# zdebruine/RcppML

Hardware: AMD Instinct MI355X
Metric: ALS updates/sec (cols solved/s), k=64 sparse NMF (higher is better)
Workload: dtype f32; 1 GPU; configs[1]: simulateNMF 20000x100000 (x1 GPUs, column shards) 1%-dense CSC, k=64, MSE, coordinate-descent NNLS (cd_maxit=100, cd_tol=1e-8), L1 row normalisation, loss every iteration; rows=20000, cols_per_gpu=100000, nnz_per_gpu=20054852, k=64, solver=cd, cd_variant=auto, parallelism=column-shard x1

## Files before the change

### rcppml_amd/csrc/cd_placement.hip.h

```cpp
#pragma once
#include <cstdint>

namespace rk {

struct CdPlace {
    int simds;
    int rounds;
    int desc;
    int extra_top;
};

constexpr int CD_PLACE_DESC = 0x6;
constexpr int CD_PLACE_EXTRA_TOP = 0;

__host__ __device__ inline int64_t cd_place_pos(const CdPlace& pl, int g, int r) {
    return (int64_t)r * pl.simds + (((pl.desc >> r) & 1) ? pl.simds - 1 - g : g);
}
__host__ __device__ inline int64_t cd_place_extra(const CdPlace& pl, int g) { return pl.extra_top ? pl.simds - 1 - g : g; }

__host__ __device__ inline int64_t cd_place_unserp(int64_t p, int tpb, int64_t ncols) {
    const int64_t blk = p / tpb, grp = blk >> 4;
    if ((grp & 1) && (grp + 1) * 16 <= (ncols >> 7)) return (((grp << 4) + 15 - (blk & 15)) * tpb) + p % tpb;
    return p;
}

}
```

### rcppml_amd/csrc/kernels_cd_mfma.hip.h

```cpp
#pragma once
#include "kernels.hip.h"
#include "cd_placement.hip.h"

namespace rk {


struct CdStepOut { float a, nx; };

__device__ __forceinline__ float cd_max_nc(float a, float b, float inf) { return __builtin_amdgcn_fmed3f(a, b, inf); }

template <bool SIMPLE>
__device__ __forceinline__ CdStepOut cd_scalar_step(float b, float xo, float ginv, bool active, float l1_cd, float l2_cd,
                                                    float lo, float hi) {
    CdStepOut o;
    if constexpr (SIMPLE) {
        const float diff = b * ginv;
        o.a = __builtin_fmaxf(diff, -xo);
        o.nx = __builtin_fmaxf(xo + diff, 0.f);
    } else {
        float diff = b * ginv;
        diff -= l1_cd;
        diff = __builtin_fmaf(l2_cd, xo, diff);
        const float nv = xo + diff;
        const bool neg = nv < lo, up = nv > hi;
        float nx = neg ? lo : (up ? hi : nv);
        float a = neg ? lo - xo : (up ? hi - xo : diff);
        const bool on = active && (ginv > 0.f);
        a = on ? a : 0.f;
        nx = on ? nx : xo;
        o.a = a;
        o.nx = nx;
    }
    return o;
}

__host__ __device__ constexpr size_t cd_mfma_lds_bytes(int RT) {
    return RT <= 2 ? (size_t)(16 * RT) * 64 * sizeof(float4) : ((size_t)(32 * RT) * (32 * RT) + 2 * (32 * RT)) * sizeof(float);
}

template <int RT>
__device__ __forceinline__ void cd_mfma_fill_lds(const float* __restrict__ G , int k) {
    constexpr int KP = 32 * RT;
    constexpr bool PACK = RT <= 2;
    extern __shared__ __attribute__((aligned(16))) char smem_raw[];
    float* Gs = reinterpret_cast<float*>(smem_raw);
    float2* tab_s = reinterpret_cast<float2*>(Gs + KP * KP);
    float4* img = reinterpret_cast<float4*>(smem_raw);
    {
        auto gp = [&](int col, int row) { return (row < k && col < k) ? G[(int64_t)col * k + row] : (row == col ? 1.f : 0.f); };
        if constexpr (PACK) {
            for (int e = threadIdx.x; e < (KP / 2) * 64; e += blockDim.x) {
                const int pr = e >> 6, w6 = e & 63;
                const int i = 2 * pr + (w6 >> 5), r = w6 & 31;
                const int h = (r >> 2) & 1, v = (r & 3) + 4 * (r >> 3);
                const float gd = gp(i, i);
                float4 t;
                t.x = -gp(i, 2 * v + h);
                t.y = RT == 2 ? -gp(i, 32 + 2 * v + h) : 0.f;
                t.z = gd > 0.f ? 1.f / gd : 0.f;
                t.w = (i & 1) ? gp(i - 1, i) : 0.f;
                img[e] = t;
            }
        } else {
            for (int e = threadIdx.x; e < KP * KP; e += blockDim.x) {
                const int pr = e >> 6, w6 = e & 63;
                const int i = 2 * (pr / RT) + (w6 >> 5), rt = pr % RT, r = w6 & 31;
                const int h = (r >> 2) & 1, v = (r & 3) + 4 * (r >> 3);
                Gs[e] = -gp(i, 32 * rt + 2 * v + h);
            }
            for (int i = threadIdx.x; i < KP; i += blockDim.x) {
                float2 t;
                const float gd = gp(i, i);
                t.x = gd > 0.f ? 1.f / gd : 0.f;
                t.y = (i & 1) ? gp(i - 1, i) : 0.f;
                tab_s[i] = t;
            }
        }
    }
}

template <int RT, int CT, bool SIMPLE>
__device__ __forceinline__ void cd_mfma_tile(const int64_t base, const float* __restrict__ B, float* __restrict__ X, int k, int64_t ncols,
                                             float l1_pre, int warm, int zero_init, float l1_cd, float l2_cd, int nonneg, int maxit,
                                             float tol, float ub_cd, float ub_post, int* __restrict__ sweeps,
                                             const int* __restrict__ order, unsigned long long* __restrict__ stats) {
    constexpr int KP = 32 * RT;
    constexpr bool PACK = RT <= 2;
    constexpr float XSIGN = SIMPLE ? -1.f : 1.f;
    extern __shared__ __attribute__((aligned(16))) char smem_raw[];
    float* Gs = reinterpret_cast<float*>(smem_raw);
    float2* tab_s = reinterpret_cast<float2*>(Gs + KP * KP);
    float4* img = reinterpret_cast<float4*>(smem_raw);
    const int lane = threadIdx.x & 63;
    const int half = lane >> 5, cl = lane & 31;
    if (base >= ncols) return;
    int64_t j[CT];
    bool inb[CT];
#pragma unroll
    for (int ct = 0; ct < CT; ++ct) {
        const int64_t slot = base + ct * 32 + cl;
        inb[ct] = slot < ncols;
        j[ct] = (inb[ct] && order) ? order[slot] : slot;
    }
    f32x16 acc[RT][CT];
    float xr[RT][CT][16];
#pragma unroll
    for (int rt = 0; rt < RT; ++rt)
#pragma unroll
        for (int ct = 0; ct < CT; ++ct) {
            const float* bj = B + j[ct] * (int64_t)k;
            const float* xj = X + j[ct] * (int64_t)k;
#pragma unroll
            for (int v = 0; v < 16; ++v) {
                const int row = 32 * rt + 2 * v + half;
                const bool ok = inb[ct] && row < k;
                float bv = ok ? bj[row] : 0.f;
                if (ok && l1_pre != 0.f) bv -= l1_pre;
                acc[rt][ct][v] = bv;
                xr[rt][ct][v] = (ok && !zero_init) ? XSIGN * xj[row] : 0.f;
            }
        }
    struct PairOps { float av[RT]; float ginv, coup; };
    auto load_pair = [&](int p) {
        PairOps o;
        if constexpr (PACK) {
            const float4 t = img[p * 64 + lane];
            o.av[0] = t.x;
            if constexpr (RT == 2) o.av[1] = t.y;
            o.ginv = t.z; o.coup = t.w;
        } else {
#pragma unroll
            for (int rt2 = 0; rt2 < RT; ++rt2) o.av[rt2] = Gs[(p * RT + rt2) * 64 + lane];
            const float2 t = tab_s[2 * p + half];
            o.ginv = t.x; o.coup = t.y;
        }
        return o;
    };
    if (warm) {
#pragma unroll
        for (int rt = 0; rt < RT; ++rt)
#pragma unroll
            for (int q = 0; q < 16; ++q) {
                const int i = 32 * rt + 2 * q;
                const PairOps po = load_pair(i >> 1);
#pragma unroll
                for (int rt2 = 0; rt2 < RT; ++rt2) {
#pragma unroll
                    for (int ct = 0; ct < CT; ++ct)
                        acc[rt2][ct] = __builtin_amdgcn_mfma_f32_32x32x2f32(po.av[rt2], XSIGN * xr[rt][ct][q], acc[rt2][ct], 0, 0, 0);
                }
            }
    }
    const float lo = nonneg ? 0.f : -INFINITY;
    const float hi = ub_cd > 0.f ? ub_cd : INFINITY;
    const bool check = tol > 0.f;
    const float inv_k = 1.f / static_cast<float>(k);
    bool active[CT];
    int nsweep[CT];
#pragma unroll
    for (int ct = 0; ct < CT; ++ct) { active[ct] = inb[ct]; nsweep[ct] = 0; }
    PairOps cur = load_pair(0);
    for (int it = 0; it < maxit; ++it) {
        bool any_active = false;
#pragma unroll
        for (int ct = 0; ct < CT; ++ct) any_active |= active[ct];
        if (!__any(any_active)) break;
        float tsum[CT];
#pragma unroll
        for (int ct = 0; ct < CT; ++ct) { tsum[ct] = 0.f; nsweep[ct] += active[ct] ? 1 : 0; }
#pragma unroll
        for (int rt = 0; rt < RT; ++rt)
#pragma unroll
            for (int q = 0; q < 16; ++q) {
                constexpr int KPc = KP;
                const int inext = (32 * rt + 2 * q + 2) % KPc;
                const int rtn = (q == 15 ? rt + 1 : rt) % RT;
                const PairOps nxt = load_pair(inext >> 1);
                const float g_oe = cur.coup;
                float aval[CT];
#pragma unroll
                for (int ct = 0; ct < CT; ++ct) {
                    const float b = acc[rt][ct][q];
                    const float xo = xr[rt][ct][q];
                    if constexpr (SIMPLE) {
                        const float ginv = cur.ginv;
                        float ae_lo = cd_max_nc(b * ginv, xo, hi);
                        asm volatile("s_nop 1\n\tv_permlane32_swap_b32 %0, %0" : "+v"(ae_lo));
                        const float bo = __builtin_fmaf(-g_oe, ae_lo, b);
                        const float diff = bo * ginv;
                        const float a = cd_max_nc(diff, xo, hi);
                        const float nxn = __builtin_fminf(xo - diff, 0.f);
                        aval[ct] = a;
                        xr[rt][ct][q] = nxn;
                        tsum[ct] = __builtin_fmaf(tabs(a), __builtin_amdgcn_rcpf(tabs(nxn) + 1e-15f), tsum[ct]);
                    } else {
                        const float ginv = cur.ginv;
                        const CdStepOut e = cd_scalar_step<SIMPLE>(b, xo, ginv, active[ct], l1_cd, l2_cd, lo, hi);
                        float ae_lo = e.a;
                        asm volatile("s_nop 1\n\tv_permlane32_swap_b32 %0, %0" : "+v"(ae_lo));
                        const float bo = __builtin_fmaf(-g_oe, ae_lo, b);
                        const CdStepOut o = cd_scalar_step<SIMPLE>(bo, xo, ginv, active[ct], l1_cd, l2_cd, lo, hi);
                        aval[ct] = o.a;
                        xr[rt][ct][q] = o.nx;
                        tsum[ct] = __builtin_fmaf(tabs(o.a), __builtin_amdgcn_rcpf(tabs(o.nx) + 1e-15f), tsum[ct]);
                    }
                }
#pragma unroll
                for (int s2 = 0; s2 < RT; ++s2) {
                    const int rt2 = (rtn + s2) % RT;
#pragma unroll
                    for (int ct = 0; ct < CT; ++ct)
                        acc[rt2][ct] = __builtin_amdgcn_mfma_f32_32x32x2f32(cur.av[rt2], aval[ct], acc[rt2][ct], 0, 0, 0);
                }
                cur = nxt;
                __builtin_amdgcn_sched_barrier(0);
            }
        bool froze = false;
#pragma unroll
        for (int ct = 0; ct < CT; ++ct) {
            const float tot = tsum[ct] + __shfl_xor(tsum[ct], 32, 64);
            const bool now = active[ct] && !(check && tot * inv_k < tol);
            froze |= active[ct] && !now;
            active[ct] = now;
        }
        if constexpr (SIMPLE) {
            if (__any(froze)) {
#pragma unroll
                for (int rt = 0; rt < RT; ++rt)
#pragma unroll
                    for (int ct = 0; ct < CT; ++ct)
#pragma unroll
                        for (int v = 0; v < 16; ++v) acc[rt][ct][v] = active[ct] ? acc[rt][ct][v] : 0.f;
            }
        }
    }
#pragma unroll
    for (int ct = 0; ct < CT; ++ct) {
        if (!inb[ct]) continue;
        float* xj = X + j[ct] * (int64_t)k;
#pragma unroll
        for (int rt = 0; rt < RT; ++rt)
#pragma unroll
            for (int v = 0; v < 16; ++v) {
                const int row = 32 * rt + 2 * v + half;
                if (row < k) {
                    float val = SIMPLE ? 0.f - xr[rt][ct][v] : xr[rt][ct][v];
                    if (ub_post > 0.f) val = val < ub_post ? val : ub_post;
                    xj[row] = val;
                }
            }
        if (sweeps && half == 0) sweeps[j[ct]] = nsweep[ct];
    }
    int nsw = 0, ncol = 0;
#pragma unroll
    for (int ct = 0; ct < CT; ++ct)
        if (inb[ct] && half == 0) { nsw += nsweep[ct]; ncol += 1; }
    cd_stats_add(stats, nsw, ncol);
}

template <int RT, int CT, bool SIMPLE>
__global__ __launch_bounds__(256) __attribute__((amdgpu_waves_per_eu((CT == 1 && RT <= 2) ? 4 : 2, 8))) void cd_mfma_kernel(const float* __restrict__ G ,
                                                       const float* __restrict__ B,
                                                       float* __restrict__ X, int k, int64_t ncols, float l1_pre,
                                                       int warm, int zero_init, float l1_cd, float l2_cd, int nonneg,
                                                       int maxit, float tol, float ub_cd, float ub_post,
                                                       int* __restrict__ sweeps, const int* __restrict__ order,
                                                       unsigned long long* __restrict__ stats) {
    cd_mfma_fill_lds<RT>(G, k);
    __syncthreads();
    const int wave = threadIdx.x >> 6;
    const int64_t base = ((int64_t)blockIdx.x * (blockDim.x >> 6) + wave) * (32 * CT);
    cd_mfma_tile<RT, CT, SIMPLE>(base, B, X, k, ncols, l1_pre, warm, zero_init, l1_cd, l2_cd, nonneg, maxit, tol, ub_cd, ub_post, sweeps,
                                 order, stats);
}

template <int RT, bool SIMPLE>
__global__ __launch_bounds__(1024) __attribute__((amdgpu_waves_per_eu(4, 8))) void cd_mfma_placed_kernel(
    const float* __restrict__ G, const float* __restrict__ B, float* __restrict__ X, int k, int64_t ncols, float l1_pre, int warm,
    int zero_init, float l1_cd, float l2_cd, int nonneg, int maxit, float tol, float ub_cd, float ub_post, int* __restrict__ sweeps,
    const int* __restrict__ order, unsigned long long* __restrict__ stats, CdPlace pl, int unserp) {
    cd_mfma_fill_lds<RT>(G, k);
    __syncthreads();
    const int w = __builtin_amdgcn_readfirstlane(threadIdx.x >> 6);
    const int g = 4 * (int)blockIdx.x + (w & 3), r = w >> 2;
    const int64_t ntiles = (ncols + 31) / 32;
    const int64_t mapped = (int64_t)pl.rounds * pl.simds;
    int64_t p = cd_place_pos(pl, g, r);
    int64_t e = r == pl.rounds - 1 ? cd_place_extra(pl, g) : ntiles;
    while (p < ntiles) {
        const int64_t t = unserp ? cd_place_unserp(p, 4, ncols) : p;
        cd_mfma_tile<RT, 1, SIMPLE>(t * 32, B, X, k, ncols, l1_pre, warm, zero_init, l1_cd, l2_cd, nonneg, maxit, tol, ub_cd, ub_post,
                                    sweeps, order, stats);
        p = mapped + e;
        e += pl.simds;
    }
}

}
```

### rcppml_amd/csrc/kernels_cd_mfma64.hip.h

```cpp
#pragma once
#include "kernels.hip.h"
#include "cd_placement.hip.h"

namespace rk {

template <class T> struct Vec4T;
template <> struct Vec4T<float> { typedef float4 type; };
template <> struct Vec4T<double> { typedef double4 type; };
template <int P> __device__ __forceinline__ unsigned bcast_row32(unsigned a) {
    if constexpr (P == 2) {
        return __builtin_amdgcn_permlane16_swap(a, a, false, false)[0];
    } else {
        const auto tu = __builtin_amdgcn_permlane16_swap(a, a, false, false);
        if constexpr (P == 0) {
            return __builtin_amdgcn_permlane32_swap(tu[0], tu[0], false, false)[0];
        } else {
            return __builtin_amdgcn_permlane32_swap(tu[1], tu[1], false, false)[0];
        }
    }
}
template <int P> __device__ __forceinline__ float bcast_row(float a) {
    return __uint_as_float(bcast_row32<P>(__float_as_uint(a)));
}
template <int P> __device__ __forceinline__ double bcast_row(double a) {
    const unsigned long long u = __double_as_longlong(a);
    const unsigned lo = bcast_row32<P>((unsigned)u), hi = bcast_row32<P>((unsigned)(u >> 32));
    return __longlong_as_double(((unsigned long long)hi << 32) | lo);
}

template <class T> struct CdStepOut64 { T a, nx; };
__device__ __forceinline__ float tmax(float a, float b) { return __builtin_fmaxf(a, b); }
__device__ __forceinline__ double tmax(double a, double b) { return __builtin_fmax(a, b); }

template <bool SIMPLE, class T>
__device__ __forceinline__ CdStepOut64<T> cd_step64(T b, T xo, T gd, T ginv, bool active, T l1_cd, T l2_cd, T lo, T hi) {
    CdStepOut64<T> o;
    if constexpr (SIMPLE) {
        const T diff = cd_quotient(b, gd, ginv);
        o.a = tmax(diff, -xo);
        o.nx = tmax(xo + diff, T(0));
    } else {
        T diff = cd_quotient(b, gd, ginv);
        diff -= l1_cd;
        diff = tfma(l2_cd, xo, diff);
        const T nv = xo + diff;
        const bool neg = nv < lo, up = nv > hi;
        T nx = neg ? lo : (up ? hi : nv);
        T a = neg ? lo - xo : (up ? hi - xo : diff);
        const bool on = active && (ginv > T(0));
        o.a = on ? a : T(0);
        o.nx = on ? nx : xo;
    }
    return o;
}

__device__ __forceinline__ f64x4 mfma16(double a, double b, f64x4 c) { return __builtin_amdgcn_mfma_f64_16x16x4f64(a, b, c, 0, 0, 0); }
typedef float f32x4 __attribute__((ext_vector_type(4)));
__device__ __forceinline__ f32x4 mfma16(float a, float b, f32x4 c) { return __builtin_amdgcn_mfma_f32_16x16x4f32(a, b, c, 0, 0, 0); }
template <class T> struct Acc4T;
template <> struct Acc4T<float> { typedef f32x4 type; };
template <> struct Acc4T<double> { typedef f64x4 type; };
__device__ __forceinline__ float fast_recip(float den) { return __builtin_amdgcn_rcpf(den); }
__device__ __forceinline__ double fast_recip(double den) {
    const double rc = __builtin_amdgcn_rcp(den);
    return __builtin_fma(__builtin_fma(-den, rc, 1.0), rc, rc);
}

template <class T, int NT>
__device__ __forceinline__ void cd_mfma64_fill_lds(const T* __restrict__ G , int k) {
    typedef typename Vec4T<T>::type Tab4;
    constexpr int KP = 16 * NT;
    extern __shared__ __attribute__((aligned(16))) char smem_raw[];
    T* Gs = reinterpret_cast<T*>(smem_raw);
    Tab4* tab_s = reinterpret_cast<Tab4*>(Gs + KP * KP);
    [[maybe_unused]] T* gd_s = Gs + KP * KP + 4 * KP;
    {
        constexpr bool PERM = sizeof(T) == 4;
        auto gp = [&](int col, int row) { return (row < k && col < k) ? G[(int64_t)col * k + row] : (row == col ? T(1) : T(0)); };
        for (int e = threadIdx.x; e < KP * KP; e += blockDim.x) {
            const int qt = e >> 6, kk = (e >> 4) & 3, ps = e & 15;
            const int q = qt / NT, t = qt % NT;
            const int rl = PERM ? (ps >> 2) + 4 * (ps & 3) : ps;
            Gs[e] = -gp(4 * q + kk, 16 * t + rl);
        }
        for (int c = threadIdx.x; c < KP; c += blockDim.x) {
            const int gg = c & 3, qb = c & ~3;
            Tab4 v;
            const T gd = gp(c, c);
            v.x = gd > T(0) ? T(1) / gd : T(0);
            v.y = gg > 0 ? gp(qb + 0, c) : T(0);
            v.z = gg > 1 ? gp(qb + 1, c) : T(0);
            v.w = gg > 2 ? gp(qb + 2, c) : T(0);
            tab_s[c] = v;
            if constexpr (sizeof(T) == 8) gd_s[c] = gd > T(0) ? gd : T(0);
        }
    }
}

template <class T, int NT, bool SIMPLE>
__device__ __forceinline__ void cd_mfma64_tile(const int64_t base, const T* __restrict__ B, T* __restrict__ X, int k, int64_t ncols, T l1_pre,
                                               int warm, int zero_init, T l1_cd, T l2_cd, int nonneg, int maxit, T tol, T ub_cd, T ub_post,
                                               int* __restrict__ sweeps, const int* __restrict__ order,
                                               unsigned long long* __restrict__ stats) {
    typedef typename Vec4T<T>::type Tab4;
    typedef typename Acc4T<T>::type Acc4;
    constexpr int KP = 16 * NT;
    extern __shared__ __attribute__((aligned(16))) char smem_raw[];
    T* Gs = reinterpret_cast<T*>(smem_raw);
    Tab4* tab_s = reinterpret_cast<Tab4*>(Gs + KP * KP);
    [[maybe_unused]] T* gd_s = Gs + KP * KP + 4 * KP;
    const int lane = threadIdx.x & 63;
    const int g = lane >> 4, cl = lane & 15;
    if (base >= ncols) return;
    const int64_t slot = base + cl;
    const bool inb = slot < ncols;
    const int64_t j = (inb && order) ? order[slot] : slot;
    Acc4 acc[NT];
    T xr[NT][4];
    {
        const T* bj = B + j * (int64_t)k;
        const T* xj = X + j * (int64_t)k;
#pragma unroll
        for (int t = 0; t < NT; ++t)
#pragma unroll
            for (int v = 0; v < 4; ++v) {
                const int row = 16 * t + 4 * v + g;
                const bool ok = inb && row < k;
                T bv = ok ? bj[row] : T(0);
                if (ok && l1_pre != T(0)) bv -= l1_pre;
                acc[t][v] = bv;
                xr[t][v] = (ok && !zero_init) ? xj[row] : T(0);
            }
    }
    if (warm) {
#pragma unroll
        for (int t = 0; t < NT; ++t)
#pragma unroll
            for (int v = 0; v < 4; ++v) {
                const int q = 4 * t + v;
#pragma unroll
                for (int t2 = 0; t2 < NT; ++t2) {
                    const T av = Gs[((q * NT + t2) << 6) + lane];
                    acc[t2] = mfma16(av, xr[t][v], acc[t2]);
                }
            }
    }
    const T lo = nonneg ? T(0) : -INFINITY;
    const T hi = ub_cd > T(0) ? ub_cd : INFINITY;
    const bool check = tol > T(0);
    const T inv_k = T(1) / static_cast<T>(k);
    bool active = inb;
    int nsweep = 0;
    Tab4 tb_c = tab_s[g];
    [[maybe_unused]] T gd_c = T(0);
    if constexpr (sizeof(T) == 8) gd_c = gd_s[g];
    T av_c[NT];
#pragma unroll
    for (int t2 = 0; t2 < NT; ++t2) av_c[t2] = Gs[(t2 << 6) + lane];
    for (int it = 0; it < maxit; ++it) {
        if (!__any(active)) break;
        T tsum = T(0);
        nsweep += active ? 1 : 0;
#pragma unroll
        for (int t = 0; t < NT; ++t)
#pragma unroll
            for (int v = 0; v < 4; ++v) {
                constexpr int NQ = KP / 4;
                const int qn = (4 * t + v + 1) % NQ;
                const int tn = (v == 3 ? t + 1 : t) % NT;
                const Tab4 tb_n = tab_s[4 * qn + g];
                [[maybe_unused]] T gd_n = T(0);
                if constexpr (sizeof(T) == 8) gd_n = gd_s[4 * qn + g];
                T av_n[NT];
#pragma unroll
                for (int t2 = 0; t2 < NT; ++t2) av_n[t2] = Gs[((qn * NT + t2) << 6) + lane];
                const T b0 = acc[t][v];
                const T xo = xr[t][v];
                const T ginv = SIMPLE ? (active ? tb_c.x : T(0)) : tb_c.x;
                const CdStepOut64<T> s0 = cd_step64<SIMPLE, T>(b0, xo, gd_c, ginv, active, l1_cd, l2_cd, lo, hi);
                const T b1 = tfma(-tb_c.y, bcast_row<0>(s0.a), b0);
                const CdStepOut64<T> s1 = cd_step64<SIMPLE, T>(b1, xo, gd_c, ginv, active, l1_cd, l2_cd, lo, hi);
                const T b2 = tfma(-tb_c.z, bcast_row<1>(s1.a), b1);
                const CdStepOut64<T> s2 = cd_step64<SIMPLE, T>(b2, xo, gd_c, ginv, active, l1_cd, l2_cd, lo, hi);
                const T b3 = tfma(-tb_c.w, bcast_row<2>(s2.a), b2);
                const CdStepOut64<T> s3 = cd_step64<SIMPLE, T>(b3, xo, gd_c, ginv, active, l1_cd, l2_cd, lo, hi);
                xr[t][v] = s3.nx;
                tsum = tfma(tabs(s3.a), fast_recip(tabs(s3.nx) + T(1e-15)), tsum);
#pragma unroll
                for (int s = 0; s < NT; ++s) {
                    const int t2 = (tn + s) % NT;
                    acc[t2] = mfma16(av_c[t2], s3.a, acc[t2]);
                }
                tb_c = tb_n;
                gd_c = gd_n;
#pragma unroll
                for (int t2 = 0; t2 < NT; ++t2) av_c[t2] = av_n[t2];
                __builtin_amdgcn_sched_barrier(0);
            }
        T tot = tsum + __shfl_xor(tsum, 16, 64);
        tot += __shfl_xor(tot, 32, 64);
        active = active && !(check && tot * inv_k < tol);
    }
    if (inb) {
        T* xj = X + j * (int64_t)k;
#pragma unroll
        for (int t = 0; t < NT; ++t)
#pragma unroll
            for (int v = 0; v < 4; ++v) {
                const int row = 16 * t + 4 * v + g;
                if (row < k) {
                    T val = xr[t][v];
                    if (ub_post > T(0)) val = val < ub_post ? val : ub_post;
                    xj[row] = val;
                }
            }
        if (sweeps && g == 0) sweeps[j] = nsweep;
    }
    cd_stats_add(stats, (inb && g == 0) ? nsweep : 0, (inb && g == 0) ? 1 : 0);
}

template <class T, int NT, bool SIMPLE>
__global__ __launch_bounds__(256) __attribute__((amdgpu_waves_per_eu(NT <= 2 ? 4 : (NT <= 4 ? 2 : 1), 8)))
void cd_mfma64_kernel(const T* __restrict__ G , const T* __restrict__ B,
                      T* __restrict__ X, int k, int64_t ncols, T l1_pre, int warm, int zero_init, T l1_cd,
                      T l2_cd, int nonneg, int maxit, T tol, T ub_cd, T ub_post,
                      int* __restrict__ sweeps, const int* __restrict__ order, unsigned long long* __restrict__ stats) {
    cd_mfma64_fill_lds<T, NT>(G, k);
    __syncthreads();
    const int wave = threadIdx.x >> 6;
    const int64_t base = ((int64_t)blockIdx.x * (blockDim.x >> 6) + wave) * 16;
    cd_mfma64_tile<T, NT, SIMPLE>(base, B, X, k, ncols, l1_pre, warm, zero_init, l1_cd, l2_cd, nonneg, maxit, tol, ub_cd, ub_post, sweeps, order,
                                  stats);
}

template <int NT, bool SIMPLE>
__global__ __launch_bounds__(512) __attribute__((amdgpu_waves_per_eu(NT <= 2 ? 4 : 2, 8)))
void cd_mfma64_placed_kernel(const float* __restrict__ G, const float* __restrict__ B, float* __restrict__ X, int k, int64_t ncols,
                             float l1_pre, int warm, int zero_init, float l1_cd, float l2_cd, int nonneg, int maxit, float tol, float ub_cd,
                             float ub_post, int* __restrict__ sweeps, const int* __restrict__ order, unsigned long long* __restrict__ stats,
                             CdPlace pl, int unserp) {
    cd_mfma64_fill_lds<float, NT>(G, k);
    __syncthreads();
    const int w = __builtin_amdgcn_readfirstlane(threadIdx.x >> 6);
    const int gs = 4 * (int)blockIdx.x + (w & 3), r = w >> 2;
    const int64_t ntiles = (ncols + 15) / 16;
    const int64_t mapped = (int64_t)pl.rounds * pl.simds;
    int64_t p = cd_place_pos(pl, gs, r);
    int64_t e = r == pl.rounds - 1 ? cd_place_extra(pl, gs) : ntiles;
    while (p < ntiles) {
        const int64_t t = unserp ? cd_place_unserp(p, 8, ncols) : p;
        cd_mfma64_tile<float, NT, SIMPLE>(t * 16, B, X, k, ncols, l1_pre, warm, zero_init, l1_cd, l2_cd, nonneg, maxit, tol, ub_cd, ub_post,
                                          sweeps, order, stats);
        p = mapped + e;
        e += pl.simds;
    }
}

}
```

### rcppml_amd/csrc/solve_cd_impl.hip.h

```cpp
#pragma once
#include <cmath>
#include "solve_common.hip.h"
#include "kernels_cd_mfma.hip.h"
#include "kernels_cd_mfma64.hip.h"
template <class T, int KP>
static void cd_lane_launch(rcppml_hip_ctx* c, const T* Gp, const T* invd, const T* B, T* X, int k,
                           int64_t ncols, T l1_pre, int warm, int zero_init, T l1_cd, T l2_cd, int nonneg,
                           int maxit, T tol, T ub_cd, T ub_post, int* sweeps, const int* order) {
    constexpr bool EXACT = std::is_same<T, double>::value;
    const int64_t nblk = (ncols + 63) / 64;
    hipLaunchKernelGGL((cd_lane_kernel<T, KP, EXACT>), dim3((unsigned)nblk), dim3(64), 0, c->stream, Gp, invd,
                       B, X, k, ncols, l1_pre, warm, zero_init, l1_cd, l2_cd, nonneg, maxit, tol, ub_cd, ub_post, sweeps, order, c->stats);
    HIPCHK(hipGetLastError());
}
template <class T, int KP, bool GLDS = true>
static void cd_wave_launch(rcppml_hip_ctx* c, const T* Gp, const T* invd, const T* B, T* X, int k,
                           int64_t ncols, T l1_pre, int warm, int zero_init, T l1_cd, T l2_cd, int nonneg,
                           int maxit, T tol, T ub_cd, T ub_post, int* sweeps, const int* order) {
    constexpr bool EXACT = std::is_same<T, double>::value;
    const size_t smem = GLDS ? (size_t)KP * KP * sizeof(T) : 0;
    auto kern = cd_wave_kernel<T, KP, EXACT, GLDS>;
    static DynSmemOnce once;
    once.ensure(reinterpret_cast<const void*>(kern), smem, c->device);
    int per_cu = (int)((160 * 1024) / (smem + 256));
    if (per_cu > 8) per_cu = 8;
    if (per_cu < 1) per_cu = 1;
    int64_t nblk = (int64_t)c->num_cu * per_cu;
    const int64_t need = (ncols + 3) / 4;
    if (nblk > need) nblk = need;
    if (nblk < 1) nblk = 1;
    hipLaunchKernelGGL(kern, dim3((unsigned)nblk), dim3(256), smem, c->stream, Gp, invd, B, X, k, ncols, l1_pre,
                       warm, zero_init, l1_cd, l2_cd, nonneg, maxit, tol, ub_cd, ub_post, sweeps, order, c->stats);
    HIPCHK(hipGetLastError());
}


template <class T, int KP, int LPC>
static void cd_group_launch(rcppml_hip_ctx* c, const T* Gp, const T* invd, const T* B, T* X, int k, int64_t ncols,
                            T l1_pre, int warm, int zero_init, T l1_cd, T l2_cd, int nonneg, int maxit, T tol, T ub_cd,
                            T ub_post, int* sweeps, const int* order) {
    constexpr bool EXACT = std::is_same<T, double>::value;
    const size_t smem = ((size_t)KP * KP + 2 * KP) * sizeof(T);
    auto kern = cd_group_kernel<T, KP, LPC, EXACT>;
    static DynSmemOnce once;
    once.ensure(reinterpret_cast<const void*>(kern), smem, c->device);
    const int64_t per_block = (int64_t)4 * (64 / LPC);
    const int64_t nblk = (ncols + per_block - 1) / per_block;
    hipLaunchKernelGGL(kern, dim3((unsigned)nblk), dim3(256), smem, c->stream, Gp, invd, B, X, k, ncols, l1_pre, warm,
                       zero_init, l1_cd, l2_cd, nonneg, maxit, tol, ub_cd, ub_post, sweeps, order, c->stats);
    HIPCHK(hipGetLastError());
}

template <int RT>
static void cd_mfma_placed_launch(rcppml_hip_ctx* c, int cus, const float* G, const float* B, float* X, int k, int64_t ncols,
                                  float l1_pre, int warm, int zero_init, float l1_cd, float l2_cd, int nonneg, int maxit, float tol,
                                  float ub_cd, float ub_post, int* sweeps, const int* order) {
    const int64_t ntiles = (ncols + 31) / 32;
    CdPlace pl;
    pl.simds = 4 * cus;
    const int64_t per = ntiles / pl.simds;
    pl.rounds = per < 1 ? 1 : (per > 4 ? 4 : (int)per);
    pl.desc = CD_PLACE_DESC;
    pl.extra_top = CD_PLACE_EXTRA_TOP;
    size_t smem = cd_mfma_lds_bytes(RT);
    const size_t alone = (size_t)160 * 1024 / 2 + 1024;
    if (smem < alone) smem = alone;
    const bool simple = nonneg && ub_cd <= 0.f && l1_cd == 0.f && l2_cd == 0.f;
    static DynSmemOnce once_simple, once_general;
    if (simple) once_simple.ensure(reinterpret_cast<const void*>(&cd_mfma_placed_kernel<RT, true>), smem, c->device);
    else once_general.ensure(reinterpret_cast<const void*>(&cd_mfma_placed_kernel<RT, false>), smem, c->device);
    const dim3 grid((unsigned)cus), block(256u * (unsigned)pl.rounds);
    if (simple)
        hipLaunchKernelGGL((cd_mfma_placed_kernel<RT, true>), grid, block, smem, c->stream, G, B, X, k, ncols, l1_pre, warm, zero_init,
                           l1_cd, l2_cd, nonneg, maxit, tol, ub_cd, ub_post, sweeps, order, c->stats, pl, order ? 1 : 0);
    else
        hipLaunchKernelGGL((cd_mfma_placed_kernel<RT, false>), grid, block, smem, c->stream, G, B, X, k, ncols, l1_pre, warm, zero_init,
                           l1_cd, l2_cd, nonneg, maxit, tol, ub_cd, ub_post, sweeps, order, c->stats, pl, order ? 1 : 0);
    HIPCHK(hipGetLastError());
}

template <int RT, int CT>
static void cd_mfma_launch(rcppml_hip_ctx* c, const float* G, const float* , const float* B, float* X, int k,
                           int64_t ncols, float l1_pre, int warm, int zero_init, float l1_cd, float l2_cd, int nonneg,
                           int maxit, float tol, float ub_cd, float ub_post, int* sweeps, const int* order) {
    if constexpr (RT <= 2 && CT == 1) {
        int mode = c->opt_cd_placed;
        if (const char* e = exp_env("RCPPML_GPU_CD_PLACED")) mode = atoi(e);
        const int cus = c->opt_cd_assume_cus > 0 ? c->opt_cd_assume_cus : (c->num_cu > 0 ? c->num_cu : 256);
        const int64_t per = ((ncols + 31) / 32) / ((int64_t)4 * cus);
        if (mode == 1 || ((mode == 0 || mode == 3) && per >= 2 && per < 5)) {
            cd_mfma_placed_launch<RT>(c, cus, G, B, X, k, ncols, l1_pre, warm, zero_init, l1_cd, l2_cd, nonneg, maxit, tol, ub_cd, ub_post,
                                      sweeps, order);
            return;
        }
    }
    size_t smem = cd_mfma_lds_bytes(RT);
    const int64_t per_block = 4 * 32 * CT;
    const int64_t nblk = (ncols + per_block - 1) / per_block;
    const bool simple = nonneg && ub_cd <= 0.f && l1_cd == 0.f && l2_cd == 0.f;
    {
        const double per_cu = (double)nblk / (double)(c->num_cu > 0 ? c->num_cu : 256);
        int cap = 0;
        if (per_cu > 1.0 && per_cu < 4.0 && per_cu - std::floor(per_cu) < 0.5) cap = (int)std::floor(per_cu);
        if (const char* e = exp_env("RCPPML_GPU_CD_CAP")) cap = atoi(e);
        if (cap > 0) {
            const size_t lds_cu = 160 * 1024;
            const size_t want = lds_cu / (size_t)(cap + 1) + 1024;
            if (want > smem && want <= lds_cu / (size_t)cap) smem = want;
        }
    }
    static DynSmemOnce once_simple, once_general;
    if (simple) once_simple.ensure(reinterpret_cast<const void*>(&cd_mfma_kernel<RT, CT, true>), smem, c->device);
    else once_general.ensure(reinterpret_cast<const void*>(&cd_mfma_kernel<RT, CT, false>), smem, c->device);
    if (simple)
        hipLaunchKernelGGL((cd_mfma_kernel<RT, CT, true>), dim3((unsigned)nblk), dim3(256), smem, c->stream, G, B, X,
                           k, ncols, l1_pre, warm, zero_init, l1_cd, l2_cd, nonneg, maxit, tol, ub_cd, ub_post, sweeps, order, c->stats);
    else
        hipLaunchKernelGGL((cd_mfma_kernel<RT, CT, false>), dim3((unsigned)nblk), dim3(256), smem, c->stream, G, B, X,
                           k, ncols, l1_pre, warm, zero_init, l1_cd, l2_cd, nonneg, maxit, tol, ub_cd, ub_post, sweeps, order, c->stats);
    HIPCHK(hipGetLastError());
}


void rcppml_cd_lmf_dispatch(rcppml_hip_ctx* c, const float* G, const float* B, float* X, int k, int64_t ncols, float l1_pre,
                            int warm, int zero_init, int maxit, float tol, float ub_post, int* sweeps, const int* order);

template <class T, int NT>
static void cd_mfma64_launch(rcppml_hip_ctx* c, const T* G, const T* , const T* B, T* X, int k,
                             int64_t ncols, T l1_pre, int warm, int zero_init, T l1_cd, T l2_cd, int nonneg,
                             int maxit, T tol, T ub_cd, T ub_post, int* sweeps, const int* order) {
    constexpr int KP = 16 * NT;
    const bool simple = nonneg && ub_cd <= T(0) && l1_cd == T(0) && l2_cd == T(0);
    if constexpr (std::is_same<T, float>::value && NT <= 4) {
        int mode = c->opt_cd_placed;
        if (const char* e = exp_env("RCPPML_GPU_CD_PLACED")) mode = atoi(e);
        const int cus = c->opt_cd_assume_cus > 0 ? c->opt_cd_assume_cus : (c->num_cu > 0 ? c->num_cu : 256);
        const int64_t ntiles = (ncols + 15) / 16, simds = (int64_t)4 * cus;
        if (mode == 1 || ((mode == 0 || mode == 4) && ntiles > simds && ntiles < 2 * simds)) {
            CdPlace pl;
            pl.simds = (int)simds;
            pl.rounds = ntiles > simds ? 2 : 1;
            pl.desc = CD_PLACE_DESC;
            pl.extra_top = CD_PLACE_EXTRA_TOP;
            size_t smem = ((size_t)KP * KP + 4 * KP) * sizeof(float);
            const size_t alone = (size_t)160 * 1024 / 2 + 1024;
            if (smem < alone) smem = alone;
            static DynSmemOnce once_simple, once_general;
            if (simple) once_simple.ensure(reinterpret_cast<const void*>(&cd_mfma64_placed_kernel<NT, true>), smem, c->device);
            else once_general.ensure(reinterpret_cast<const void*>(&cd_mfma64_placed_kernel<NT, false>), smem, c->device);
            const dim3 grid((unsigned)cus), block(256u * (unsigned)pl.rounds);
            if (simple)
                hipLaunchKernelGGL((cd_mfma64_placed_kernel<NT, true>), grid, block, smem, c->stream, G, B, X, k, ncols, l1_pre, warm, zero_init,
                                   l1_cd, l2_cd, nonneg, maxit, tol, ub_cd, ub_post, sweeps, order, c->stats, pl, order ? 1 : 0);
            else
                hipLaunchKernelGGL((cd_mfma64_placed_kernel<NT, false>), grid, block, smem, c->stream, G, B, X, k, ncols, l1_pre, warm, zero_init,
                                   l1_cd, l2_cd, nonneg, maxit, tol, ub_cd, ub_post, sweeps, order, c->stats, pl, order ? 1 : 0);
            HIPCHK(hipGetLastError());
            return;
        }
    }
    const size_t smem = ((size_t)KP * KP + 4 * KP + (sizeof(T) == 8 ? KP : 0)) * sizeof(T);
    const int64_t nblk = (ncols + 63) / 64;
    static DynSmemOnce once_simple, once_general;
    if (simple) once_simple.ensure(reinterpret_cast<const void*>(&cd_mfma64_kernel<T, NT, true>), smem, c->device);
    else once_general.ensure(reinterpret_cast<const void*>(&cd_mfma64_kernel<T, NT, false>), smem, c->device);
    if (simple)
        hipLaunchKernelGGL((cd_mfma64_kernel<T, NT, true>), dim3((unsigned)nblk), dim3(256), smem, c->stream, G, B, X, k,
                           ncols, l1_pre, warm, zero_init, l1_cd, l2_cd, nonneg, maxit, tol, ub_cd, ub_post, sweeps, order, c->stats);
    else
        hipLaunchKernelGGL((cd_mfma64_kernel<T, NT, false>), dim3((unsigned)nblk), dim3(256), smem, c->stream, G, B, X, k,
                           ncols, l1_pre, warm, zero_init, l1_cd, l2_cd, nonneg, maxit, tol, ub_cd, ub_post, sweeps, order, c->stats);
    HIPCHK(hipGetLastError());
}

template <class T>
static int pick_lpc(int KP) {
    const int ev = 16 / (int)sizeof(T);
    const char* e = exp_env("RCPPML_GPU_CD_LPC");
    int lpc = e ? atoi(e) : (std::is_same<T, float>::value ? KP / 32 : KP / 16);
    if (lpc < 1) lpc = 1;
    if (lpc > 4) lpc = 4;
    while (lpc < 4 && KP / lpc > 32) lpc *= 2;
    while (lpc > 1 && (KP / lpc) % ev != 0) lpc /= 2;
    return lpc;
}

template <class T>
static void solve_cd_impl(rcppml_hip_ctx* c, const T* G, const T* B, T* X, int k, int64_t ncols, T l1_pre,
                          int warm, int zero_init, T l1_cd, T l2_cd, int nonneg, int maxit, T tol, T ub_cd,
                          T ub_post, int variant, int* sweeps, const int* order) {
    if (ncols <= 0) return;
    if (k < 1 || k > 256) throw std::runtime_error("solve_cd: k must be in [1,256]");
    if (k > 128) {
        T *Gp, *invd;
        pad_impl<T>(c, G, k, 256, &Gp, &invd);
        cd_wave_launch<T, 256, false>(c, Gp, invd, B, X, k, ncols, l1_pre, warm, zero_init, l1_cd, l2_cd, nonneg, maxit, tol, ub_cd,
                                      ub_post, sweeps, order);
        return;
    }
    int KP = solve_kp(k);
    const bool lmf_ok = std::is_same<T, float>::value && k <= 64 && nonneg && ub_cd <= T(0) && l1_cd == T(0) && l2_cd == T(0) && maxit >= 1;
    if (variant == RCPPML_CD_LMF && !lmf_ok) variant = RCPPML_CD_AUTO;
    if (variant == RCPPML_CD_AUTO && lmf_ok && k <= 32 && ncols >= (int64_t)256 * c->num_cu && !c->opt_cd_no_lmf &&
        !exp_env("RCPPML_GPU_CD_VARIANT"))
        variant = RCPPML_CD_LMF;
    if (variant == RCPPML_CD_LMF) {
        if constexpr (std::is_same<T, float>::value)
            rcppml_cd_lmf_dispatch(c, G, B, X, k, ncols, l1_pre, warm, zero_init, maxit, tol, ub_post, sweeps, order);
        return;
    }
    if (variant == RCPPML_CD_AUTO && k <= 64 && nonneg && ub_cd <= T(0) && l1_cd == T(0) && l2_cd == T(0) && maxit >= 1 &&
        ncols <= (int64_t)6 * (c->num_cu > 0 ? c->num_cu : 256) && !exp_env("RCPPML_GPU_CD_VARIANT")) {
        const unsigned nblk = (unsigned)((ncols + 3) / 4);
        if (k <= 16)
            hipLaunchKernelGGL((cd_wave_static_kernel<T, 16>), dim3(nblk), dim3(256), 0, c->stream, G, B, X, k, ncols, l1_pre, warm, zero_init,
                               maxit, tol, ub_post, sweeps, c->stats);
        else if (k <= 32)
            hipLaunchKernelGGL((cd_wave_static_kernel<T, 32>), dim3(nblk), dim3(256), 0, c->stream, G, B, X, k, ncols, l1_pre, warm, zero_init,
                               maxit, tol, ub_post, sweeps, c->stats);
        else
            hipLaunchKernelGGL((cd_wave_static_kernel<T, 64>), dim3(nblk), dim3(256), 0, c->stream, G, B, X, k, ncols, l1_pre, warm, zero_init,
                               maxit, tol, ub_post, sweeps, c->stats);
        HIPCHK(hipGetLastError());
        return;
    }
    if (variant == RCPPML_CD_AUTO) {
        const char* e = exp_env("RCPPML_GPU_CD_VARIANT");
        if (e && !strcmp(e, "lane")) variant = RCPPML_CD_LANE;
        else if (e && !strcmp(e, "wave")) variant = RCPPML_CD_WAVE;
        else if (e && !strcmp(e, "group")) variant = RCPPML_CD_GROUP;
        else if (e && !strcmp(e, "mfma")) variant = RCPPML_CD_MFMA;
        else if (e && !strcmp(e, "mfma16")) variant = RCPPML_CD_MFMA16;
        else variant = RCPPML_CD_MFMA;
        if (variant == RCPPML_CD_MFMA && std::is_same<T, float>::value && k <= 64 && !e) {
            static int small16 = -1;
            if (small16 < 0) small16 = exp_flag("RCPPML_GPU_CD_SMALL16", "0") ? 0 : 1;
            if (small16 && (ncols + 31) / 32 < (int64_t)4 * c->num_cu) variant = RCPPML_CD_MFMA16;
        }
    }
    if (variant == RCPPML_CD_MFMA && !std::is_same<T, float>::value) variant = RCPPML_CD_MFMA16;
    if (variant == RCPPML_CD_MFMA16 && k > 64 && std::is_same<T, float>::value) variant = RCPPML_CD_MFMA;
    if (variant == RCPPML_CD_MFMA) KP = 32 * ((k + 31) / 32);
    if (variant == RCPPML_CD_MFMA16) KP = 16 * ((k + 15) / 16);
    const int lane_max = std::is_same<T, float>::value ? 64 : 32;
    if (variant == RCPPML_CD_LANE && KP > lane_max) variant = RCPPML_CD_GROUP;
    if (variant != RCPPML_CD_LANE && variant != RCPPML_CD_WAVE && variant != RCPPML_CD_MFMA && variant != RCPPML_CD_MFMA16) variant = RCPPML_CD_GROUP;
    if (variant == RCPPML_CD_WAVE && KP < 64) KP = 64;
    T *Gp = const_cast<T*>(G), *invd = nullptr;
    if (variant != RCPPML_CD_MFMA && variant != RCPPML_CD_MFMA16) pad_impl<T>(c, G, k, KP, &Gp, &invd);
#define CD_ARGS c, Gp, invd, B, X, k, ncols, l1_pre, warm, zero_init, l1_cd, l2_cd, nonneg, maxit, tol, ub_cd, ub_post, sweeps, order
    if (variant == RCPPML_CD_LANE) {
        switch (KP) {
            case 16: cd_lane_launch<T, 16>(CD_ARGS); break;
            case 32: cd_lane_launch<T, 32>(CD_ARGS); break;
            default:
                if constexpr (std::is_same<T, float>::value) cd_lane_launch<T, 64>(CD_ARGS);
                break;
        }
    } else if (variant == RCPPML_CD_MFMA) {
        if constexpr (std::is_same<T, float>::value) {
            switch (KP) {
                case 32: cd_mfma_launch<1, 1>(CD_ARGS); break;
                case 64: cd_mfma_launch<2, 1>(CD_ARGS); break;
                case 96: cd_mfma_launch<3, 1>(CD_ARGS); break;
                default: cd_mfma_launch<4, 1>(CD_ARGS); break;
            }
        }
    } else if (variant == RCPPML_CD_MFMA16) {
        switch (KP) {
            case 16: cd_mfma64_launch<T, 1>(CD_ARGS); break;
            case 32: cd_mfma64_launch<T, 2>(CD_ARGS); break;
            case 48: cd_mfma64_launch<T, 3>(CD_ARGS); break;
            case 64: cd_mfma64_launch<T, 4>(CD_ARGS); break;
            default:
                if constexpr (std::is_same<T, double>::value) {
                    switch (KP) {
                        case 80: cd_mfma64_launch<T, 5>(CD_ARGS); break;
                        case 96: cd_mfma64_launch<T, 6>(CD_ARGS); break;
                        case 112: cd_mfma64_launch<T, 7>(CD_ARGS); break;
                        default: cd_mfma64_launch<T, 8>(CD_ARGS); break;
                    }
                } else cd_mfma64_launch<T, 4>(CD_ARGS);
                break;
        }
    } else if (variant == RCPPML_CD_GROUP) {
        const int lpc = pick_lpc<T>(KP);
#define GROUP_CASE(K_, L_) if (KP == K_ && lpc == L_) { cd_group_launch<T, K_, L_>(CD_ARGS); launched = true; }
        bool launched = false;
        GROUP_CASE(16, 1) GROUP_CASE(16, 2) GROUP_CASE(16, 4)
        GROUP_CASE(32, 1) GROUP_CASE(32, 2) GROUP_CASE(32, 4)
        GROUP_CASE(64, 2) GROUP_CASE(64, 4)
        GROUP_CASE(128, 4)
#undef GROUP_CASE
        if (!launched) throw std::runtime_error("solve_cd: no lane-group configuration for this rank");
    } else {
        if (KP == 64) cd_wave_launch<T, 64>(CD_ARGS);
        else cd_wave_launch<T, 128>(CD_ARGS);
    }
#undef CD_ARGS
}
```

Baseline: 110.6 million cols/s.

## Add mixed-width CD kernel assigning 16- and 32-column tiles per SIMD

When the number of 16-column tiles falls between one and two times the SIMD count, a new mixed kernel launches one wave per SIMD. Some waves solve a single 16-column tile with the 64-wide MFMA path, and the rest solve a 32-column tile with the 32x32 MFMA path, so every SIMD gets one wave instead of some SIMDs running two rounds. Both G images are placed in LDS at different offsets. The tolerance sum is split into two accumulators to shorten the dependency chain. This replaces the default placed two-round kernel, and the price is extra LDS, a double fill of G, and possible imbalance between waves of different widths.

```diff
diff --git a/rcppml_amd/csrc/cd_placement.hip.h b/rcppml_amd/csrc/cd_placement.hip.h
--- a/rcppml_amd/csrc/cd_placement.hip.h
+++ b/rcppml_amd/csrc/cd_placement.hip.h
@@ -24,4 +24,10 @@
     return p;
 }
 
+__host__ __device__ inline int64_t cd_mixed_p0(int64_t ntiles, int simds) { return (2 * (int64_t)simds - ntiles) & ~(int64_t)1; }
+__host__ __device__ inline int64_t cd_mixed_pos(int64_t p0, int u, bool* wide) {
+    *wide = u >= p0;
+    return *wide ? p0 + 2 * ((int64_t)u - p0) : (int64_t)u;
 }
+
+}
diff --git a/rcppml_amd/csrc/kernels_cd_mfma.hip.h b/rcppml_amd/csrc/kernels_cd_mfma.hip.h
--- a/rcppml_amd/csrc/kernels_cd_mfma.hip.h
+++ b/rcppml_amd/csrc/kernels_cd_mfma.hip.h
@@ -38,14 +38,14 @@
     return RT <= 2 ? (size_t)(16 * RT) * 64 * sizeof(float4) : ((size_t)(32 * RT) * (32 * RT) + 2 * (32 * RT)) * sizeof(float);
 }
 
-template <int RT>
+template <int RT, int LDS_OFF = 0>
 __device__ __forceinline__ void cd_mfma_fill_lds(const float* __restrict__ G , int k) {
     constexpr int KP = 32 * RT;
     constexpr bool PACK = RT <= 2;
     extern __shared__ __attribute__((aligned(16))) char smem_raw[];
-    float* Gs = reinterpret_cast<float*>(smem_raw);
+    float* Gs = reinterpret_cast<float*>(smem_raw + LDS_OFF);
     float2* tab_s = reinterpret_cast<float2*>(Gs + KP * KP);
-    float4* img = reinterpret_cast<float4*>(smem_raw);
+    float4* img = reinterpret_cast<float4*>(smem_raw + LDS_OFF);
     {
         auto gp = [&](int col, int row) { return (row < k && col < k) ? G[(int64_t)col * k + row] : (row == col ? 1.f : 0.f); };
         if constexpr (PACK) {
@@ -79,7 +79,7 @@
     }
 }
 
-template <int RT, int CT, bool SIMPLE>
+template <int RT, int CT, bool SIMPLE, int LDS_OFF = 0, bool TOL4 = false>
 __device__ __forceinline__ void cd_mfma_tile(const int64_t base, const float* __restrict__ B, float* __restrict__ X, int k, int64_t ncols,
                                              float l1_pre, int warm, int zero_init, float l1_cd, float l2_cd, int nonneg, int maxit,
                                              float tol, float ub_cd, float ub_post, int* __restrict__ sweeps,
@@ -88,9 +88,9 @@
     constexpr bool PACK = RT <= 2;
     constexpr float XSIGN = SIMPLE ? -1.f : 1.f;
     extern __shared__ __attribute__((aligned(16))) char smem_raw[];
-    float* Gs = reinterpret_cast<float*>(smem_raw);
+    float* Gs = reinterpret_cast<float*>(smem_raw + LDS_OFF);
     float2* tab_s = reinterpret_cast<float2*>(Gs + KP * KP);
-    float4* img = reinterpret_cast<float4*>(smem_raw);
+    float4* img = reinterpret_cast<float4*>(smem_raw + LDS_OFF);
     const int lane = threadIdx.x & 63;
     const int half = lane >> 5, cl = lane & 31;
     if (base >= ncols) return;
@@ -165,9 +165,14 @@
 #pragma unroll
         for (int ct = 0; ct < CT; ++ct) any_active |= active[ct];
         if (!__any(any_active)) break;
-        float tsum[CT];
-#pragma unroll
-        for (int ct = 0; ct < CT; ++ct) { tsum[ct] = 0.f; nsweep[ct] += active[ct] ? 1 : 0; }
+        constexpr int NTS = TOL4 ? 2 : 1;
+        float tsum[CT][NTS];
+#pragma unroll
+        for (int ct = 0; ct < CT; ++ct) {
+#pragma unroll
+            for (int ts = 0; ts < NTS; ++ts) tsum[ct][ts] = 0.f;
+            nsweep[ct] += active[ct] ? 1 : 0;
+        }
 #pragma unroll
         for (int rt = 0; rt < RT; ++rt)
 #pragma unroll
@@ -176,6 +181,7 @@
                 const int inext = (32 * rt + 2 * q + 2) % KPc;
                 const int rtn = (q == 15 ? rt + 1 : rt) % RT;
                 const PairOps nxt = load_pair(inext >> 1);
+                const int ts = TOL4 ? (q & 1) : 0;
                 const float g_oe = cur.coup;
                 float aval[CT];
 #pragma unroll
@@ -192,7 +198,7 @@
                         const float nxn = __builtin_fminf(xo - diff, 0.f);
                         aval[ct] = a;
                         xr[rt][ct][q] = nxn;
-                        tsum[ct] = __builtin_fmaf(tabs(a), __builtin_amdgcn_rcpf(tabs(nxn) + 1e-15f), tsum[ct]);
+                        tsum[ct][ts] = __builtin_fmaf(tabs(a), __builtin_amdgcn_rcpf(tabs(nxn) + 1e-15f), tsum[ct][ts]);
                     } else {
                         const float ginv = cur.ginv;
                         const CdStepOut e = cd_scalar_step<SIMPLE>(b, xo, ginv, active[ct], l1_cd, l2_cd, lo, hi);
@@ -202,7 +208,7 @@
                         const CdStepOut o = cd_scalar_step<SIMPLE>(bo, xo, ginv, active[ct], l1_cd, l2_cd, lo, hi);
                         aval[ct] = o.a;
                         xr[rt][ct][q] = o.nx;
-                        tsum[ct] = __builtin_fmaf(tabs(o.a), __builtin_amdgcn_rcpf(tabs(o.nx) + 1e-15f), tsum[ct]);
+                        tsum[ct][ts] = __builtin_fmaf(tabs(o.a), __builtin_amdgcn_rcpf(tabs(o.nx) + 1e-15f), tsum[ct][ts]);
                     }
                 }
 #pragma unroll
@@ -218,7 +224,8 @@
         bool froze = false;
 #pragma unroll
         for (int ct = 0; ct < CT; ++ct) {
-            const float tot = tsum[ct] + __shfl_xor(tsum[ct], 32, 64);
+            float tot = tsum[ct][0] + __shfl_xor(tsum[ct][0], 32, 64);
+            if constexpr (TOL4) tot += tsum[ct][1] + __shfl_xor(tsum[ct][1], 32, 64);
             const bool now = active[ct] && !(check && tot * inv_k < tol);
             froze |= active[ct] && !now;
             active[ct] = now;
diff --git a/rcppml_amd/csrc/kernels_cd_mfma64.hip.h b/rcppml_amd/csrc/kernels_cd_mfma64.hip.h
--- a/rcppml_amd/csrc/kernels_cd_mfma64.hip.h
+++ b/rcppml_amd/csrc/kernels_cd_mfma64.hip.h
@@ -66,12 +66,12 @@
     return __builtin_fma(__builtin_fma(-den, rc, 1.0), rc, rc);
 }
 
-template <class T, int NT>
+template <class T, int NT, int LDS_OFF = 0>
 __device__ __forceinline__ void cd_mfma64_fill_lds(const T* __restrict__ G , int k) {
     typedef typename Vec4T<T>::type Tab4;
     constexpr int KP = 16 * NT;
     extern __shared__ __attribute__((aligned(16))) char smem_raw[];
-    T* Gs = reinterpret_cast<T*>(smem_raw);
+    T* Gs = reinterpret_cast<T*>(smem_raw + LDS_OFF);
     Tab4* tab_s = reinterpret_cast<Tab4*>(Gs + KP * KP);
     [[maybe_unused]] T* gd_s = Gs + KP * KP + 4 * KP;
     {
@@ -97,7 +97,7 @@
     }
 }
 
-template <class T, int NT, bool SIMPLE>
+template <class T, int NT, bool SIMPLE, int LDS_OFF = 0>
 __device__ __forceinline__ void cd_mfma64_tile(const int64_t base, const T* __restrict__ B, T* __restrict__ X, int k, int64_t ncols, T l1_pre,
                                                int warm, int zero_init, T l1_cd, T l2_cd, int nonneg, int maxit, T tol, T ub_cd, T ub_post,
                                                int* __restrict__ sweeps, const int* __restrict__ order,
@@ -106,7 +106,7 @@
     typedef typename Acc4T<T>::type Acc4;
     constexpr int KP = 16 * NT;
     extern __shared__ __attribute__((aligned(16))) char smem_raw[];
-    T* Gs = reinterpret_cast<T*>(smem_raw);
+    T* Gs = reinterpret_cast<T*>(smem_raw + LDS_OFF);
     Tab4* tab_s = reinterpret_cast<Tab4*>(Gs + KP * KP);
     [[maybe_unused]] T* gd_s = Gs + KP * KP + 4 * KP;
     const int lane = threadIdx.x & 63;
diff --git a/rcppml_amd/csrc/kernels_cd_mixed.hip.h b/rcppml_amd/csrc/kernels_cd_mixed.hip.h
--- /dev/null
+++ b/rcppml_amd/csrc/kernels_cd_mixed.hip.h
@@ -0,0 +1,35 @@
+#pragma once
+#include "kernels_cd_mfma.hip.h"
+#include "kernels_cd_mfma64.hip.h"
+
+namespace rk {
+
+__host__ __device__ constexpr int cd_mixed_lds_off(int NT) { return (16 * NT * 16 * NT + 4 * 16 * NT) * (int)sizeof(float); }
+__host__ __device__ constexpr int cd_mixed_rt(int NT) { return NT <= 2 ? 1 : 2; }
+__host__ __device__ constexpr size_t cd_mixed_lds_bytes(int NT) { return (size_t)cd_mixed_lds_off(NT) + cd_mfma_lds_bytes(cd_mixed_rt(NT)); }
+
+template <int NT, bool SIMPLE>
+__global__ __launch_bounds__(256) __attribute__((amdgpu_waves_per_eu(2, 8)))
+void cd_mfma_mixed_kernel(const float* __restrict__ G, const float* __restrict__ B, float* __restrict__ X, int k, int64_t ncols,
+                          float l1_pre, int warm, int zero_init, float l1_cd, float l2_cd, int nonneg, int maxit, float tol, float ub_cd,
+                          float ub_post, int* __restrict__ sweeps, const int* __restrict__ order, unsigned long long* __restrict__ stats,
+                          int64_t p0, int unserp) {
+    constexpr int RT = cd_mixed_rt(NT);
+    constexpr int OFF = cd_mixed_lds_off(NT);
+    static_assert(OFF % 16 == 0, "the 32-column image holds float4");
+    cd_mfma64_fill_lds<float, NT>(G, k);
+    cd_mfma_fill_lds<RT, OFF>(G, k);
+    __syncthreads();
+    const int w = __builtin_amdgcn_readfirstlane(threadIdx.x >> 6);
+    bool wide;
+    const int64_t p = cd_mixed_pos(p0, 4 * (int)blockIdx.x + w, &wide);
+    const int64_t t = unserp ? cd_place_unserp(p, 8, ncols) : p;
+    if (wide)
+        cd_mfma_tile<RT, 1, SIMPLE, OFF, true>(t * 16, B, X, k, ncols, l1_pre, warm, zero_init, l1_cd, l2_cd, nonneg, maxit, tol, ub_cd,
+                                               ub_post, sweeps, order, stats);
+    else
+        cd_mfma64_tile<float, NT, SIMPLE>(t * 16, B, X, k, ncols, l1_pre, warm, zero_init, l1_cd, l2_cd, nonneg, maxit, tol, ub_cd, ub_post,
+                                          sweeps, order, stats);
+}
+
+}
diff --git a/rcppml_amd/csrc/solve_cd_impl.hip.h b/rcppml_amd/csrc/solve_cd_impl.hip.h
--- a/rcppml_amd/csrc/solve_cd_impl.hip.h
+++ b/rcppml_amd/csrc/solve_cd_impl.hip.h
@@ -3,6 +3,7 @@
 #include "solve_common.hip.h"
 #include "kernels_cd_mfma.hip.h"
 #include "kernels_cd_mfma64.hip.h"
+#include "kernels_cd_mixed.hip.h"
 template <class T, int KP>
 static void cd_lane_launch(rcppml_hip_ctx* c, const T* Gp, const T* invd, const T* B, T* X, int k,
                            int64_t ncols, T l1_pre, int warm, int zero_init, T l1_cd, T l2_cd, int nonneg,
@@ -88,7 +89,7 @@
         if (const char* e = exp_env("RCPPML_GPU_CD_PLACED")) mode = atoi(e);
         const int cus = c->opt_cd_assume_cus > 0 ? c->opt_cd_assume_cus : (c->num_cu > 0 ? c->num_cu : 256);
         const int64_t per = ((ncols + 31) / 32) / ((int64_t)4 * cus);
-        if (mode == 1 || ((mode == 0 || mode == 3) && per >= 2 && per < 5)) {
+        if (mode == 1 || ((mode == 0 || mode == 3 || mode == 5) && per >= 2 && per < 5)) {
             cd_mfma_placed_launch<RT>(c, cus, G, B, X, k, ncols, l1_pre, warm, zero_init, l1_cd, l2_cd, nonneg, maxit, tol, ub_cd, ub_post,
                                       sweeps, order);
             return;
@@ -136,7 +137,26 @@
         if (const char* e = exp_env("RCPPML_GPU_CD_PLACED")) mode = atoi(e);
         const int cus = c->opt_cd_assume_cus > 0 ? c->opt_cd_assume_cus : (c->num_cu > 0 ? c->num_cu : 256);
         const int64_t ntiles = (ncols + 15) / 16, simds = (int64_t)4 * cus;
-        if (mode == 1 || ((mode == 0 || mode == 4) && ntiles > simds && ntiles < 2 * simds)) {
+        const bool between = ntiles > simds && ntiles < 2 * simds;
+        if (mode == 0 && between) {
+            size_t smem = cd_mixed_lds_bytes(NT);
+            const size_t alone = (size_t)160 * 1024 / 2 + 1024;
+            if (smem < alone) smem = alone;
+            const int64_t p0 = cd_mixed_p0(ntiles, (int)simds);
+            static DynSmemOnce once_simple, once_general;
+            if (simple) once_simple.ensure(reinterpret_cast<const void*>(&cd_mfma_mixed_kernel<NT, true>), smem, c->device);
+            else once_general.ensure(reinterpret_cast<const void*>(&cd_mfma_mixed_kernel<NT, false>), smem, c->device);
+            const dim3 grid((unsigned)cus), block(256u);
+            if (simple)
+                hipLaunchKernelGGL((cd_mfma_mixed_kernel<NT, true>), grid, block, smem, c->stream, G, B, X, k, ncols, l1_pre, warm, zero_init,
+                                   l1_cd, l2_cd, nonneg, maxit, tol, ub_cd, ub_post, sweeps, order, c->stats, p0, order ? 1 : 0);
+            else
+                hipLaunchKernelGGL((cd_mfma_mixed_kernel<NT, false>), grid, block, smem, c->stream, G, B, X, k, ncols, l1_pre, warm, zero_init,
+                                   l1_cd, l2_cd, nonneg, maxit, tol, ub_cd, ub_post, sweeps, order, c->stats, p0, order ? 1 : 0);
+            HIPCHK(hipGetLastError());
+            return;
+        }
+        if (mode == 1 || ((mode == 4 || mode == 5) && between)) {
             CdPlace pl;
             pl.simds = (int)simds;
             pl.rounds = ntiles > simds ? 2 : 1;
```

Measured after the change: 109.8 million cols/s. About the same (-0.7%).
